# IPMI-ICNS-UKE/4d-cbct-mc

Hardware: AMD Instinct MI355X
Metric: photon histories/sec (512^3 vol, 894 proj) (higher is better)
Workload: dtype f32

## Files before the change

4d-cbct-mc_amd/csrc/engine.cpp:

```cpp
#include "engine_internal.hpp"

using namespace mcgpu;

namespace mcgpu {
namespace {
thread_local std::string g_last_error;
}
int set_error(int code, const std::string& msg) {
  g_last_error = msg.find("ERROR") == std::string::npos ? "!!ERROR!! " + msg : msg;
  return code;
}
}

extern "C" {

int mcgpu_abi_version(void) { return 1; }
void mcgpu_set_last_error_(const char* message) { (void)set_error(-1, message ? message : "unknown failure"); }
const char* mcgpu_last_error(void) { return g_last_error.c_str(); }

int mcgpu_create(const char* input_path, int device_id, mcgpu_ctx** out) {
  ABI_BEGIN
  require(input_path && out, -1, "!!ERROR!! mcgpu_create: null argument");
  knobs_warn_unknown();
  std::unique_ptr<mcgpu_ctx> c(new mcgpu_ctx);
// ... 58 lines not shown
  else if (k == "bricks_exterior") *value = ctx->dev.bricks_exterior;
  else if (k == "exterior_cylinder") *value = ctx->dev.ell_inv[0] > 0.f ? 1 : 0;
  else if (k == "sub_bricks") *value = (long long)ctx->dev.sub_n[0] * ctx->dev.sub_n[1] * ctx->dev.sub_n[2];
  else if (k == "sub_bricks_mixed") *value = ctx->dev.sub_mixed;
  else if (k == "tile_records") *value = ctx->dev.tile_rec ? 1 : 0;
  else if (k == "sub_brick_table") *value = ctx->dev.sub ? 1 : 0;
  else if (k == "segment_loop") *value = make_args(*ctx, 0).segment_loop;
  else if (k == "fast_scheduler") *value = ctx->dev.knobs.fast_sched;
  else if (k == "tiles_in_mixed_bricks") *value = ctx->dev.tiles_in_mixed_bricks;
  else if (k == "warp_field_bytes") *value = (long long)ctx->dev.warp_field_bytes;
  else if (k == "warp_field_buffer") *value = ctx->dev.dvf ? 1 : 0;
  else if (k == "correspondence_dims") *value = ctx->dev.corr_coef ? ctx->dev.corr_k : 0;
  else if (k == "blocks_per_cu") *value = ctx->dev.resident_fast;
  else if (k == "lds_bytes_fast") *value = ctx->dev.lds.total;
  else if (k == "tally_stage_bins") *value = stage_wanted(ctx->dev) ? (long long)ctx->dev.stage_bins : 0;
  else if (k == "tally_stage_capacity") *value = ctx->dev.stage_plan.cap;
  else if (k == "tally_stage_bytes") *value = (long long)ctx->dev.stage_region_bytes;
  else if (k == "tally_stage_fallback_hits") {
    unsigned long long n = 0;
    if (ctx->has_device && ctx->dev.stage_fallback) {
      HIP_TRY(hipSetDevice(ctx->dev.device_id));
      HIP_TRY(hipDeviceSynchronize());
      HIP_TRY(hipMemcpy(&n, ctx->dev.stage_fallback, 8, hipMemcpyDeviceToHost));
    }
    *value = (long long)n;
  }
  else if (k == "tally_stage_staged_hits") {
    unsigned long long n = 0;
    const size_t words = (size_t)ctx->dev.stage_plan.workgroups * ctx->dev.stage_plan.n_bins;
    if (ctx->has_device && ctx->dev.stage_counts && words != 0) {
      std::vector<unsigned int> c(words);
      HIP_TRY(hipSetDevice(ctx->dev.device_id));
      HIP_TRY(hipDeviceSynchronize());
      HIP_TRY(hipMemcpy(c.data(), ctx->dev.stage_counts, words * 4, hipMemcpyDeviceToHost));
      for (unsigned int v : c) n += v;
    }
    *value = (long long)n;
  }
// ... 67 lines not shown
  if (total_histories) *total_histories = L.total_histories;
  return 0;
  ABI_END
}

int mcgpu_advance_seed(int batch_number, unsigned long long total_histories, int seed) {
  return ranecu_advance_seed(batch_number, total_histories, seed);
}

static bool stage_wanted(const DeviceModel& D) {
  if (D.stage_cursor < 0 || D.knobs.tally_stage == 0) return false;
  if (D.knobs.tally_stage > 0) return true;
  return D.brick_count > 0 && 100LL * D.bricks_exterior >= (long long)kStageExteriorPercent * D.brick_count;
}

static void stage_prepare(mcgpu_ctx& C, TrackArgs& A, int blocks, hipStream_t stream) {
  DeviceModel& D = C.dev;
  if (D.stage_alloc_failed || blocks <= 0) return;
  const TallyStagePlan P = tally_stage_plan(4ULL * (unsigned long long)C.host.detector[0].total_pixels, A.count, (unsigned int)blocks, D.stage_bins,
                                            (unsigned int)D.knobs.stage_cap);
  if (P.n_bins == 0u || P.n_bins != D.stage_bins) return;
  const size_t counts_bytes = (size_t)blocks * P.n_bins * 4;
  try {
    if (!D.stage_fallback) D.stage_fallback = D.put(std::vector<unsigned long long>(2, 0ULL));
    if (counts_bytes > D.stage_counts_bytes) {
      if (D.stage_counts) { D.mem.free(D.stage_counts); D.stage_counts = nullptr; D.stage_counts_bytes = 0; }
      D.stage_counts = (unsigned int*)D.mem.device_bytes(counts_bytes);
      D.stage_counts_bytes = counts_bytes;
    }
    if (P.bytes > D.stage_region_bytes) {
      if (D.stage_region) { D.mem.free(D.stage_region); D.stage_region = nullptr; D.stage_region_bytes = 0; }
      D.stage_region = (unsigned long long*)D.mem.device_bytes((size_t)P.bytes);
      D.stage_region_bytes = (size_t)P.bytes;
    }
  } catch (const Error&) {
    (void)hipGetLastError();
    D.stage_alloc_failed = true;
    return;
  }
  StageArgs S{};
  S.region = D.stage_region; S.counts = D.stage_counts; S.fallback = D.stage_fallback;
  S.pixels = P.pixels; S.n_bins = P.n_bins; S.magic = P.magic; S.bin_pixels = P.bin_pixels; S.cap = P.cap;
  S.cursor = D.stage_cursor;
  if (!D.stage_fold_ready) {
    HIP_TRY(prepare_tally_fold(S));
    D.stage_fold_ready = true;
  }
  HIP_TRY(hipMemsetAsync(D.stage_counts, 0, counts_bytes, stream));
  D.stage_plan = P;
  A.stage = S;
}

int mcgpu_tally_stage_plan(const mcgpu_ctx* ctx, unsigned long long detector_words, unsigned long long histories, int workgroups, int bins,
                           unsigned long long limit, unsigned long long* out6) {
  ABI_BEGIN
  (void)ctx;
  require(out6 && workgroups > 0 && bins >= 0 && limit > 0, -1, "!!ERROR!! mcgpu_tally_stage_plan: bad argument");
  const TallyStagePlan P = tally_stage_plan(detector_words, std::min(histories, limit), (unsigned int)workgroups, (unsigned int)bins, 0u);
  out6[0] = P.n_bins; out6[1] = P.words_per_bin; out6[2] = P.bin_pixels; out6[3] = P.cap; out6[4] = P.bytes;
  out6[5] = stage_sub_launches(histories, limit);
  return 0;
  ABI_END
}

int mcgpu_tally_stage_map(unsigned long long detector_words, int bins, unsigned long long first, unsigned long long n, unsigned int* bin_out,
                          unsigned int* rel_out) {
  ABI_BEGIN
  require(bin_out && rel_out && bins >= 0 && first + n <= detector_words, -1, "!!ERROR!! mcgpu_tally_stage_map: bad argument");
  const TallyStagePlan P = tally_stage_plan(detector_words, 1, 1, (unsigned int)bins, 0u);
  require(P.n_bins != 0u, -2, "!!ERROR!! mcgpu_tally_stage_map: no staging plan for this detector");
  for (unsigned long long i = 0; i < n; ++i) {
    stage_map((unsigned int)(first + i), P.pixels, P.n_bins, P.magic, P.bin_pixels, bin_out[i], rel_out[i]);
    require(stage_unmap(bin_out[i], rel_out[i], P.pixels, P.n_bins, P.bin_pixels) == (unsigned int)(first + i), -9,
            "!!ERROR!! internal: stage_map and stage_unmap disagree");
  }
// ... 37 lines not shown
      HIP_TRY(launch_track_compat(A, (int)blocks, stream));
    } else {
      if (D.resident_fast <= 0) {
        D.resident_fast = D.knobs.blocks_per_cu > 0 ? D.knobs.blocks_per_cu : std::min(occupancy_track_fast(A), occupancy_track_fast64(A));
        if (D.resident_fast <= 0) D.resident_fast = 1;
      }
      unsigned long long resident = (unsigned long long)D.num_cus * (unsigned long long)D.resident_fast;
      resident += resident * (unsigned long long)D.knobs.grid_spare_percent / 100ULL;
      A.work_counter = D.work_counter;
      const bool staged = stage_wanted(D);
      const unsigned long long limit = staged ? D.knobs.stage_max_histories : count;
      const unsigned long long n_sub = staged ? stage_sub_launches(count, limit) : 1ULL;
      for (unsigned long long k = 0; k < n_sub; ++k) {
        stage_sub_launch(first, count, limit, k, A.first, A.count);
        const int blocks = (int)std::min((A.count + kPoolBlockThreads - 1) / kPoolBlockThreads, resident);
        HIP_TRY(hipMemsetAsync(D.work_counter, 0, (size_t)kNumCounters * kCounterStride * 8, stream));
        A.stage = StageArgs{};
        if (staged) stage_prepare(*ctx, A, blocks, stream);
        if (mode == MCGPU_MODE_FAST_STATS) {
#if defined(MC_WITH_STATS) && MC_WITH_STATS
          if (!D.stats) D.stats = D.put(std::vector<unsigned long long>(kNumStats + 3 * kWaveTrace, 0ULL));
          A.stats = D.stats;
          HIP_TRY(launch_track_stats(A, blocks, stream));
#else
          throw Error(-2, "!!ERROR!! mcgpu_launch_projection: MCGPU_MODE_FAST_STATS needs the diagnostic library (libmcgpu_amd_stats.so, MCGPU_AMD_LIB)");
#endif
        } else if (mode == MCGPU_MODE_FAST_F64) {
          HIP_TRY(launch_track_fast64(A, blocks, stream));
        } else {
          HIP_TRY(launch_track_fast(A, blocks, stream));
        }
        if (A.stage.region != nullptr) HIP_TRY(launch_tally_fold(A.stage, (unsigned int)blocks, A.image, stream));
      }
    }
  }
  HIP_TRY(hipEventRecord(D.ev_stop, stream));
  D.timed = true;
  return 0;
  ABI_END
}

int mcgpu_set_fast_schedule(mcgpu_ctx* ctx, int thresh_compton, int thresh_rayleigh, int thresh_new, int flyable_low, int swap_batch) {
  ABI_BEGIN
  require(ctx && ctx->has_device, -1, "!!ERROR!! mcgpu_set_fast_schedule: no device context");
  require(thresh_compton >= 1 && thresh_rayleigh >= 1 && thresh_new >= 1 && flyable_low >= 1 && swap_batch >= 1 && thresh_compton <= 64 &&
              thresh_rayleigh <= 64 && thresh_new <= 64 && flyable_low <= 64 && swap_batch <= 64,
          -2, "!!ERROR!! mcgpu_set_fast_schedule: thresholds are lane counts in 1..64");
// ... 313 lines not shown
```

4d-cbct-mc_amd/csrc/engine_internal.hpp:

```cpp
#pragma once
#include <hip/hip_runtime.h>

#include <algorithm>
#include <chrono>
#include <cstdarg>
#include <cstdio>
#include <cmath>
#include <cstring>
#include <map>
#include <memory>
#include <string>
#include <unordered_map>

#include "../../include/mcgpu_amd.h"
#include "knobs.hpp"
#include "device_model.hpp"
#include "ascii_device.hpp"
#include "geometry_device.hpp"
#include "image_map.hpp"

namespace mcgpu {

hipError_t launch_track_compat(const TrackArgs& args, int blocks, hipStream_t stream);
hipError_t launch_track_fast(const TrackArgs& args, int blocks, hipStream_t stream);
int occupancy_track_fast(const TrackArgs& args);
hipError_t launch_track_fast64(const TrackArgs& args, int blocks, hipStream_t stream);
int occupancy_track_fast64(const TrackArgs& args);
hipError_t launch_kat_fast64(int n, const unsigned int* u, const double* a, const double* b, const double* c, const float* dir, double* out, hipStream_t stream);
#if defined(MC_WITH_STATS) && MC_WITH_STATS
hipError_t launch_track_stats(const TrackArgs& args, int blocks, hipStream_t stream);
#endif
hipError_t prepare_tally_fold(const StageArgs& S);
hipError_t launch_tally_fold(const StageArgs& S, unsigned int workgroups, unsigned long long* image, hipStream_t stream);
hipError_t microbench_valu_issue(int num_cus, double out3[3], hipStream_t stream);
hipError_t microbench_atomic_rate(double* out, hipStream_t stream);
hipError_t microbench_copy_rate(int num_cus, double* out, hipStream_t stream);
hipError_t launch_kat_rng(int mode, int seed, int batch, int hpt, int n, float* out_dev, hipStream_t stream);
hipError_t launch_kat_streams_fast(int generator, unsigned int seed, unsigned int stream_key, unsigned long long first_id,
                                   const unsigned long long* ids_dev, int n_ids, int n_draws, unsigned int* out_dev, hipStream_t stream);
hipError_t launch_kat_math(int n, const double* x, double* l, double* e, double* s, double* c, hipStream_t stream);
hipError_t launch_kat_expf(int n, const float* x, float* e, hipStream_t stream);
hipError_t launch_kat_f32(int op, int n, const float* a, const float* b, float* out, hipStream_t stream);
hipError_t launch_warp(int nx, int ny, int nz, const unsigned char* mat, const float* dens, const float* dvf, unsigned char default_mat,
                       float default_dens, unsigned char* out_mat, float* out_dens, hipStream_t stream);
hipError_t launch_finalize(unsigned long long* image, int nx, int nz, int crop_nx, double norm, float* planes, int clear, hipStream_t stream);


int set_error(int code, const std::string& msg);
// ... 69 lines not shown
  int has_exterior = 0, bricks_exterior = 0;
  float objbox_lo[3] = {0, 0, 0}, objbox_hi[3] = {0, 0, 0};
  float ell_c[2] = {0, 0}, ell_inv[2] = {0, 0};
  LdsLayout lds;
  TrackCold* cold = nullptr;
  TrackCold cold_host;
  unsigned long long* dose_voxels = nullptr;
  unsigned long long* dose_materials = nullptr;
  size_t dose_roi_voxels = 0;
  int dose_flags = 0;
  SourcePose* src_all = nullptr;
  DetectorPose* det_all = nullptr;
  int resident_fast = 0;
  unsigned long long* stats = nullptr;
  unsigned long long* work_counter = nullptr;
  int stage_cursor = -1;
  unsigned int stage_bins = 0;
  unsigned long long* stage_region = nullptr;
  size_t stage_region_bytes = 0;
  unsigned int* stage_counts = nullptr;
  size_t stage_counts_bytes = 0;
  unsigned long long* stage_fallback = nullptr;
  bool stage_alloc_failed = false, stage_fold_ready = false;
  TallyStagePlan stage_plan{};
  unsigned long long* scratch_image = nullptr;
  float *woodcock = nullptr, *mfp = nullptr, *mfp_tot = nullptr;
  float* wood_coarse = nullptr;
  int sig_shift = -1;
  int sched[5] = {40, 12, 44, 12, 40};
  bool sched_set = false;
  struct Knobs {
    int exterior_mode = 3;
    bool compat_stats = false;
    int compat_thresh[4] = {-1, -1, -1, -1};
    int blocks_per_cu = 0;
    int grid_spare_percent = 0;
    int sched_override[5] = {-1, -1, -1, -1, -1};
    int slot_trade = 3, hold_q = 6;
// ... 64 lines not shown
```

4d-cbct-mc_amd/csrc/knobs.cpp:

```cpp
#include <cstdio>
#include <cstdlib>
#include <cstring>
#include <mutex>
#include <string>

#include "host_model.hpp"
#include "knobs.hpp"
#include "../../include/mcgpu_amd.h"

extern char** environ;

namespace mcgpu {

const KnobSpec kKnobs[] = {
    {"MCGPU_AMD_LIB", 's', 'P', "4d-cbct-mc_amd/libmcgpu_amd.so", "library the Python mirror loads (engine.py: load_library); A/B builds and the diagnostic library go through it"},
    {"MCGPU_FAST_SCHED", 'i', 'K', "0", "FAST scheduler: 0 per-wave pools, 1 workgroup-level pool (bit-identical, 14-23 % slower; fixed when the model is uploaded)"},
    {"MCGPU_SEGMENT_LOOP", 'i', 'K', "-1", "flight segment as an inner loop: 1 on, 0 off, -1 host heuristic (tile records, or >= 20 electron shells per material on average)"},
    {"MCGPU_TILE_RECORDS", 'i', 'K', "auto", "16-byte tile records (two to four palette entries + a 64-bit mask per 4x4x4 tile) as second level of the u8 volume: 1 on, 0 off; default on when the tiles of the mixed bricks exceed 8 MiB (thorax +9 %, CT-textured +29 %); identical tallies"},
    {"MCGPU_SUB_BRICKS", 'i', 'K', "0", "4-bit sub-brick codes as second level (superseded by the tile records; kept for A/B)"},
    {"MCGPU_MAX_BRICKS", 'i', 'K', "fit", "upper limit of the LDS brick grid (a coarser grid frees LDS); default: what is left of 80 KB after the tables"},
    {"MCGPU_NO_BRACKETS", 'b', 'K', "off", "no cross-section brackets in LDS: every material change asks the exact table"},
    {"MCGPU_NO_EXTERIOR", 'b', 'K', "off", "no analytic exterior hop / source entry: delta-tracking everywhere, as the reference"},
    {"MCGPU_EXTERIOR_MODE", 'i', 'K', "3", "bit 0: exterior hop of photons in flight, bit 1: analytic source entry"},
    {"MCGPU_NO_ELLIPSE", 'b', 'K', "off", "object region = bounding box only (no elliptic cylinder; default: cylinder when >= 5 % of the bricks lie outside it)"},
    {"MCGPU_THRESH_COMPTON", 'i', 'K', "40", "lanes a Compton batch waits for (1..64); setting any schedule knob also switches the scan's autotune off"},
    {"MCGPU_THRESH_RAYLEIGH", 'i', 'K', "12", "lanes a Rayleigh batch waits for"},
    {"MCGPU_THRESH_NEW", 'i', 'K', "44", "lanes a tally + source batch waits for"},
    {"MCGPU_FLYABLE_LOW", 'i', 'K', "12", "below this many flyable histories the wave drains its pending kinds"},
    {"MCGPU_SWAP_BATCH", 'i', 'K', "40", "lanes that may park before the next scheduling point"},
    {"MCGPU_HOLD_Q", 'i', 'K', "6", "a flight segment ends when all but hold_q/16 of its starting lanes have parked (0..15)"},
    {"MCGPU_SLOT_TRADE", 'i', 'K', "3", "bit 0: trade slots for flyable histories, bit 1: for the service batches"},
    {"MCGPU_NO_AUTOTUNE", 'b', 'K', "off", "scan driver: keep the default schedule instead of probing the three presets on 6e6 histories"},
    {"MCGPU_BLOCKS_PER_CU", 'i', 'K', "occupancy", "resident FAST workgroups per CU (default: what the occupancy query reports, normally 2)"},
    {"MCGPU_GRID_SPARE_PERCENT", 'i', 'K', "0", "extra workgroups beyond the resident grid, in percent"},
    {"MCGPU_TALLY_STAGE", 'i', 'K', "-1", "FAST kernels: detector hits are staged per (workgroup, bin) with plain stores and folded into the image by a second kernel (tally_fold.hip) instead of one 64-bit atomic each (bit-identical): 1 on, 0 off, -1 on where at least 50 % of the bricks are exterior (`bricks_exterior` / `brick_count`: Catphan 96 % +3 %; CIRS 26 %, thorax 43 %: 1.7-6 % slower, left on the atomics) ; in every setting only where the cursor table ((bins + 1) x 4 B) fits what the LDS image leaves of 80 KB -- otherwise the launch runs the direct atomics, also when forced on (`geti(\"tally_stage_bins\")` = 0 says so)"},
    {"MCGPU_TALLY_STAGE_MAX_HISTORIES", 'i', 'K', "134217728", "staged launches above this many histories are split into sub-launches, each followed by its fold (the staging buffer takes about 10 bytes per history of a sub-launch)"},
    {"MCGPU_COMPAT_THRESH_COMPTON", 'i', 'K', "-1", "COMPAT kernel: lanes a Compton batch waits for (-1: built-in 32, or 48 when the materials average >= 20 electron shells)"},
    {"MCGPU_COMPAT_THRESH_RAYLEIGH", 'i', 'K', "-1", "COMPAT kernel: Rayleigh batch threshold (built-in 4 / 8)"},
    {"MCGPU_COMPAT_THRESH_NEW", 'i', 'K', "-1", "COMPAT kernel: tally + source batch threshold (built-in 24 / 16)"},
    {"MCGPU_COMPAT_THRESH_TAKE", 'i', 'K', "-1", "COMPAT kernel: lanes whose parked history could fly while their register history cannot, to exchange the two (built-in 2)"},
    {"MCGPU_COMPAT_STATS", 'i', 'K', "0", "COMPAT kernel section counters (diagnostic build -DMC_COMPAT_STATS only)"},
    {"MCGPU_IGNORE_VOXBIN", 'b', 'H', "off", "parse geometry.vox(.gz) even when a newer geometry.voxbin sidecar lies beside it"},
    {"MCGPU_ASCII_HOST", 'b', 'H', "off", "format the reference's ASCII projection files on the host threads instead of the device (A/B)"},
    {"MCGPU_ASCII_WRITERS", 'i', 'H', "slots", "ASCII files in flight (1..MCGPU_ASCII_SLOTS)"},
    {"MCGPU_PINNED_COHERENT", 'b', 'H', "off", "coherent pinned host buffers for the downloads (default: non-coherent)"},
    {"MCGPU_FDK_DIRECT_RAMP", 'b', 'H', "off", "FDK ramp filter as a direct LDS convolution instead of hipFFT"},
    {"MCGPU_CORRESPONDENCE_SLAB", 'i', 'H', "4194304", "device fit of a correspondence model: field elements per slab (T slabs of 4 bytes per element are staged on the device at a time)"},
    {"MCGPU_REDUCE", 's', 'H', "auto", "multi-device tally sum: `rccl` = one ncclReduce per projection; default: tally exchange, else projection sharding"},
    {"MCGPU_RCCL_LIBRARY", 's', 'H', "librccl.so.1", "RCCL library the reduction route opens with dlopen"},
    {"MCGPU_EXCHANGE_POLICY", 'i', 'H', "1", "tally exchange: 1 the owner of a projection rotates over the ranks, 0 rank 0 owns every projection"},
// ... 57 lines not shown
```

4d-cbct-mc_amd/csrc/model_device.cpp:

```cpp
#include "engine_internal.hpp"

namespace mcgpu {

std::vector<float> coarse_woodcock(const HostModel& H) {
  const int nv = H.mat.num_values, nc = (nv + (1 << kWoodShift) - 1) >> kWoodShift;
  const double e0 = (double)H.mat.e0, de = 1.0 / (double)H.mat.ide;
  std::vector<float> out((size_t)nc, 0.f);
  for (int c = 0; c < nc; ++c) {
    double lo = 1.0e30;
    for (int i = c << kWoodShift; i < std::min(nv, (c + 1) << kWoodShift); ++i) {
      const double x = (double)H.mat.woodcock[i].x, y = (double)H.mat.woodcock[i].y;
      lo = std::min(lo, std::min(x + (e0 + i * de) * y, x + (e0 + (i + 1) * de) * y));
    }
    out[(size_t)c] = (float)(lo * (1.0 - 1.0e-6));
  }
  return out;
}

static void mark_exterior_region(const HostModel& H, DeviceModel& D, const std::vector<unsigned char>& object, bool have_background,
                                 std::vector<unsigned char>& exterior) {
  const int k = D.brick_shift, nvx[3] = {H.voxels.n[0], H.voxels.n[1], H.voxels.n[2]};
  exterior.assign((size_t)D.brick_count, 0);
  D.has_exterior = 0;
  D.bricks_exterior = 0;
// ... 757 lines not shown
      wmax = std::max(wmax, std::max((hi - m) / m, (m - lo) / m));
    }
    B.w[c] = (float)std::min(wmax * 1.001 + 1e-5, 1e30);
  }
  return B;
}

static void lay_out_lds_and_brackets(const HostModel& H, DeviceModel& D, const std::vector<float>& tot) {
  const LdsPlan P = plan_lds(H, D, D.brick_bytes);
  D.sig_shift = -1;
  if (!knob_set("MCGPU_NO_BRACKETS") && D.nmat > 0)
    for (int shift = 6; shift <= 12 && D.sig_shift < 0; ++shift)
      if (lay_out_lds(P, shift).total <= kLdsPerWorkgroup) D.sig_shift = shift;
  D.lds = lay_out_lds(P, D.sig_shift);
  {
    const TallyStagePlan S = tally_stage_plan(4ULL * (unsigned long long)H.detector[0].total_pixels, 1, 1, 0, 0);
    const int bytes = ((int)(S.n_bins + 1u) * 4 + 15) / 16 * 16;
    D.stage_cursor = -1;
    D.stage_bins = 0;
    if (S.n_bins != 0u && D.lds.total + bytes <= kLdsPerWorkgroup) {
      D.stage_cursor = D.lds.total;
      D.stage_bins = S.n_bins;
      D.lds.total += bytes;
    }
  }
  if (D.sig_shift < 0) return;
  const SigmaBrackets B = sigma_brackets(H, tot, D.nmat, D.sig_shift);
  D.cold_host.sig_mid = D.put(B.mid);
  D.cold_host.sig_w = D.put(B.w);
}

static void upload_dose_tallies(const HostModel& H, DeviceModel& D) {
  const SimConfig& cfg = H.cfg;
  if (cfg.flag_material_dose == 1) {
// ... 236 lines not shown
```

4d-cbct-mc_amd/csrc/tally_fold.hip:

```cpp
#include <hip/hip_runtime.h>

#include "tally_stage.hpp"

namespace mcgpu {
namespace {

constexpr int kFoldThreads = 1024;
extern __shared__ __attribute__((aligned(16))) unsigned long long fold_lds[];

__device__ __forceinline__ void fold_add(unsigned long long record, unsigned int words) {
  const unsigned int rel = (unsigned int)(record >> 32);
  if (rel < words) atomicAdd(fold_lds + rel, record & 0xFFFFFFFFULL);
}

__global__ __launch_bounds__(kFoldThreads) void tally_stage_fold(const StageArgs S, const unsigned int workgroups, unsigned long long* __restrict__ image) {
  const unsigned int bin = blockIdx.x, words = 4u * S.bin_pixels;
  for (unsigned int i = threadIdx.x; i < words; i += kFoldThreads) fold_lds[i] = 0ULL;
  __syncthreads();
  const unsigned int wave = (unsigned int)__builtin_amdgcn_readfirstlane((int)(threadIdx.x >> 6)), lane = threadIdx.x & 63u;
  constexpr unsigned int kWaves = kFoldThreads / 64;
  constexpr unsigned int kGroup = 4, kDeep = 4;
  for (unsigned int g0 = wave; g0 < workgroups; g0 += 64u * kWaves) {
    const unsigned int g_mine = g0 + lane * kWaves;
    const unsigned int n_mine = g_mine < workgroups ? min(S.counts[(size_t)g_mine * S.n_bins + bin], S.cap) : 0u;
    for (unsigned int l0 = 0; l0 < 64u && g0 + l0 * kWaves < workgroups; l0 += kGroup) {
      ulonglong2 r[kGroup][kDeep];
      unsigned int n[kGroup];
      const unsigned long long* src[kGroup];
#pragma unroll
      for (unsigned int u = 0; u < kGroup; ++u) {
        n[u] = (unsigned int)__builtin_amdgcn_readlane((int)n_mine, (int)(l0 + u));
        const unsigned int g = min(g0 + (l0 + u) * kWaves, workgroups - 1u);
        src[u] = S.region + (size_t)(g * S.n_bins + bin) * S.cap;
        const ulonglong2* const src2 = reinterpret_cast<const ulonglong2*>(src[u]);
#pragma unroll
        for (unsigned int j = 0; j < kDeep; ++j) {
          const unsigned int i = lane + 64u * j;
          r[u][j] = make_ulonglong2(~0ULL, ~0ULL);
          if (i < (n[u] >> 1)) r[u][j] = src2[i];
        }
      }
#pragma unroll
      for (unsigned int u = 0; u < kGroup; ++u) {
#pragma unroll
        for (unsigned int j = 0; j < kDeep; ++j) {
          fold_add(r[u][j].x, words);
          fold_add(r[u][j].y, words);
        }
        const ulonglong2* const src2 = reinterpret_cast<const ulonglong2*>(src[u]);
        for (unsigned int i = lane + 64u * kDeep; i < (n[u] >> 1); i += 64u) {
          const ulonglong2 a = src2[i];
          fold_add(a.x, words);
          fold_add(a.y, words);
        }
        if ((n[u] & 1u) != 0u && lane == 0u) fold_add(src[u][n[u] - 1u], words);
      }
    }
  }
  __syncthreads();
  for (unsigned int i = threadIdx.x; i < words; i += kFoldThreads) {
    const unsigned long long v = fold_lds[i];
    if (v == 0ULL) continue;
    const unsigned int w = stage_unmap(bin, i, S.pixels, S.n_bins, S.bin_pixels);
    if (w != 0xFFFFFFFFu) image[w] += v;
  }
}

}

hipError_t prepare_tally_fold(const StageArgs& S) {
  const size_t lds = (size_t)4 * S.bin_pixels * 8;
  if (lds <= 64 * 1024) return hipSuccess;
  return hipFuncSetAttribute(reinterpret_cast<const void*>(&tally_stage_fold), hipFuncAttributeMaxDynamicSharedMemorySize, (int)lds);
}

hipError_t launch_tally_fold(const StageArgs& S, unsigned int workgroups, unsigned long long* image, hipStream_t stream) {
  hipLaunchKernelGGL(tally_stage_fold, dim3(S.n_bins), dim3(kFoldThreads), (size_t)4 * S.bin_pixels * 8, stream, S, workgroups, image);
  return hipGetLastError();
}

}
```

4d-cbct-mc_amd/csrc/tally_stage.hpp:

```cpp
#pragma once
#include <cstdint>

#if defined(__HIPCC__)
#define MC_STAGE_HD __host__ __device__
#else
#define MC_STAGE_HD
#endif

namespace mcgpu {

constexpr unsigned int kStageRun = 64;
constexpr unsigned int kStageRunsPerBin = 64;
constexpr int kStageExteriorPercent = 50;
constexpr unsigned int kStageCapSlack = 16;
constexpr unsigned int kStageWorkgroupSlack = 2u * 16u * 256u;

struct TallyStagePlan {
  unsigned int pixels;
  unsigned int n_bins;
  unsigned int bin_pixels;
  unsigned int words_per_bin;
  unsigned int magic;
  unsigned int cap;
  unsigned int workgroups;
// ... 46 lines not shown
MC_STAGE_HD inline unsigned int stage_unmap(unsigned int bin, unsigned int rel, unsigned int pixels, unsigned int n_bins, unsigned int bin_pixels) {
  const unsigned int plane = (rel >= bin_pixels ? 1u : 0u) + (rel >= 2u * bin_pixels ? 1u : 0u) + (rel >= 3u * bin_pixels ? 1u : 0u);
  const unsigned int off = rel - plane * bin_pixels;
  const unsigned long long pixel = ((unsigned long long)(off / kStageRun) * n_bins + bin) * kStageRun + (off % kStageRun);
  return pixel < pixels ? plane * pixels + (unsigned int)pixel : 0xFFFFFFFFu;
}

inline void stage_sub_launch(unsigned long long first, unsigned long long count, unsigned long long limit, unsigned long long k, unsigned long long& sub_first,
                             unsigned long long& sub_count) {
  const unsigned long long at = k * limit;
  sub_first = first + (at < count ? at : count);
  sub_count = at < count ? (count - at < limit ? count - at : limit) : 0ULL;
}
inline unsigned long long stage_sub_launches(unsigned long long count, unsigned long long limit) { return count == 0 ? 1ULL : (count + limit - 1) / limit; }

struct StageArgs {
  unsigned long long* region;
  unsigned int* counts;
  unsigned long long* fallback;
  unsigned int pixels, n_bins, magic, bin_pixels, cap;
  int cursor;
};

}
```

4d-cbct-mc_amd/engine.py:

```python
from __future__ import annotations

import ctypes as C
import os
from pathlib import Path
from typing import Optional, Sequence

import numpy as np

MODE_FAST, MODE_COMPAT, MODE_FAST_STATS, MODE_FAST_F64 = 0, 1, 2, 3
_MODES = {"fast": MODE_FAST, "compat": MODE_COMPAT, "stats": MODE_FAST_STATS, "fast64": MODE_FAST_F64, MODE_FAST: MODE_FAST,
          MODE_COMPAT: MODE_COMPAT, MODE_FAST_STATS: MODE_FAST_STATS, MODE_FAST_F64: MODE_FAST_F64}

LIB_PATH = Path(os.environ.get("MCGPU_AMD_LIB", Path(__file__).resolve().parent / "libmcgpu_amd.so"))
EXE_PATH = Path(__file__).resolve().parent / "MC-GPU_v1.3.x"

ABI_SYMBOLS = (
    "mcgpu_abi_version", "mcgpu_knob_table", "mcgpu_last_error", "mcgpu_create", "mcgpu_clone", "mcgpu_destroy", "mcgpu_config_i64", "mcgpu_config_f64",
    "mcgpu_host_table", "mcgpu_projection_file_name", "mcgpu_image_words", "mcgpu_launch_shape", "mcgpu_advance_seed",
    "mcgpu_launch_projection", "mcgpu_tally_stage_plan", "mcgpu_tally_stage_map", "mcgpu_tally_stage_sub_launch", "mcgpu_scheduler_stats", "mcgpu_scheduler_stats_ex", "mcgpu_last_kernel_ms", "mcgpu_clear_image", "mcgpu_run_projection",
    "mcgpu_write_projection", "mcgpu_format_projection", "mcgpu_write_formatted_projection", "mcgpu_dose_info", "mcgpu_dose_read", "mcgpu_dose_clear", "mcgpu_write_dose_report",
    "mcgpu_finalize_projection", "mcgpu_finalize_projection_host", "mcgpu_stack_create", "mcgpu_stack_append", "mcgpu_stack_write_slice", "mcgpu_stack_finish",
    "mcgpu_stack_read", "mcgpu_normalize_stack", "mcgpu_run_scan", "mcgpu_run_scan_multi", "mcgpu_set_projection_angles", "mcgpu_set_geometry_arrays",
    "mcgpu_warp_volume", "mcgpu_warp_geometry", "mcgpu_map_image", "mcgpu_set_geometry_image",
    "mcgpu_correspondence_set", "mcgpu_correspondence_fit", "mcgpu_correspondence_predict", "mcgpu_warp_geometry_signal", "mcgpu_correspondence_clear",
    "mcgpu_write_voxel_file", "mcgpu_write_voxel_binary", "mcgpu_kat_rng", "mcgpu_kat_rng_streams", "mcgpu_microbench", "mcgpu_kat_math", "mcgpu_kat_expf", "mcgpu_kat_f32", "mcgpu_kat_fast64", "mcgpu_kat_tile_records", "mcgpu_fdk_reconstruct", "mcgpu_forward_project", "mcgpu_forward_project_context", "mcgpu_rooster4d_reconstruct", "mcgpu_rooster4d_stage", "mcgpu_set_fast_schedule", "mcgpu_reload_env_knobs",
    "mcgpu_exchange_shared_bytes", "mcgpu_exchange_card_bytes", "mcgpu_exchange_create", "mcgpu_exchange_card", "mcgpu_exchange_connect",
    "mcgpu_exchange_connect_local", "mcgpu_exchange_probe", "mcgpu_exchange_owner", "mcgpu_exchange_begin", "mcgpu_exchange_submit", "mcgpu_exchange_collect",
    "mcgpu_exchange_stats", "mcgpu_exchange_destroy", "mcgpu_copy_to_host",
    "mcgpu_rccl_create", "mcgpu_rccl_reduce_u64", "mcgpu_rccl_destroy",
)


class ScanOptions(C.Structure):
    _fields_ = [("struct_size", C.c_uint), ("mode", C.c_int), ("first_projection", C.c_int), ("num_projections", C.c_int),
# ... 59 lines not shown
    lib.mcgpu_knob_table.restype = C.c_size_t
    lib.mcgpu_create.argtypes = [cp, ci, C.POINTER(vp)]
    lib.mcgpu_clone.argtypes = [vp, ci, C.POINTER(vp)]
    lib.mcgpu_destroy.argtypes = [vp]
    lib.mcgpu_destroy.restype = None
    lib.mcgpu_config_i64.argtypes = [vp, cp, C.POINTER(C.c_longlong)]
    lib.mcgpu_config_f64.argtypes = [vp, cp, C.POINTER(C.c_double)]
    lib.mcgpu_host_table.argtypes = [vp, cp, C.POINTER(vp), C.POINTER(C.c_size_t)]
    lib.mcgpu_projection_file_name.argtypes = [vp, ci, cp, C.c_size_t]
    lib.mcgpu_image_words.argtypes = [vp, C.POINTER(C.c_size_t)]
    lib.mcgpu_launch_shape.argtypes = [cull, ci, ci, C.POINTER(ci), C.POINTER(ci), C.POINTER(cull)]
    lib.mcgpu_advance_seed.argtypes = [ci, cull, ci]
    lib.mcgpu_launch_projection.argtypes = [vp, ci, ci, ci, cull, cull, ci, vp, vp]
    lib.mcgpu_tally_stage_plan.argtypes = [vp, cull, cull, ci, ci, cull, C.POINTER(cull)]
    lib.mcgpu_tally_stage_map.argtypes = [cull, ci, cull, cull, vp, vp]
    lib.mcgpu_tally_stage_sub_launch.argtypes = [cull, cull, cull, cull, C.POINTER(cull), C.POINTER(cull)]
    lib.mcgpu_last_kernel_ms.argtypes = [vp, C.POINTER(C.c_float)]
    lib.mcgpu_scheduler_stats.argtypes = [vp, C.POINTER(cull), ci]
    lib.mcgpu_scheduler_stats_ex.argtypes = [vp, C.POINTER(cull), ci, ci]
    lib.mcgpu_clear_image.argtypes = [vp, vp, vp]
    lib.mcgpu_run_projection.argtypes = [vp, ci, ci, ci, cull, cull, ci, vp, C.POINTER(C.c_double), C.POINTER(cull)]
    lib.mcgpu_write_projection.argtypes = [vp, ci, vp, cull, C.c_double, cp]
    lib.mcgpu_format_projection.argtypes = [vp, vp, cull, ci, vp]
    lib.mcgpu_write_formatted_projection.argtypes = [vp, ci, ci, cull, C.c_double, cp]
    lib.mcgpu_dose_info.argtypes = [vp, C.POINTER(ci), C.POINTER(ci), C.POINTER(C.c_size_t)]
    lib.mcgpu_dose_read.argtypes = [vp, vp, vp]
    lib.mcgpu_dose_clear.argtypes = [vp]
    lib.mcgpu_write_dose_report.argtypes = [vp, vp, vp, cull, C.c_double, cp, C.c_size_t]
    lib.mcgpu_finalize_projection.argtypes = [vp, vp, cull, ci, vp, ci, vp]
    lib.mcgpu_finalize_projection_host.argtypes = [vp, vp, cull, ci, vp]
# ... 62 lines not shown


def tally_stage_plan(detector_words: int, histories: int, workgroups: int, bins: int = 0, limit: int = 1 << 27, ctx=None) -> dict:
    out = (C.c_ulonglong * 6)()
    _check(load_library().mcgpu_tally_stage_plan(ctx.h if ctx is not None else None, int(detector_words), int(histories), int(workgroups), int(bins), int(limit), out))
    return dict(zip(("bins", "words_per_bin", "bin_pixels", "capacity", "bytes", "sub_launches"), (int(v) for v in out)))


def tally_stage_map(detector_words: int, bins: int = 0, first: int = 0, n: Optional[int] = None):
    n = int(detector_words) - int(first) if n is None else int(n)
    b, r = np.empty(n, np.uint32), np.empty(n, np.uint32)
    _check(load_library().mcgpu_tally_stage_map(int(detector_words), int(bins), int(first), n, b.ctypes.data, r.ctypes.data))
    return b, r


def tally_stage_sub_launch(first: int, count: int, limit: int, k: int):
    f, c = C.c_ulonglong(), C.c_ulonglong()
    _check(load_library().mcgpu_tally_stage_sub_launch(int(first), int(count), int(limit), int(k), C.byref(f), C.byref(c)))
    return f.value, c.value


def advance_seed(batch_number: int, total_histories: int, seed: int) -> int:
    return load_library().mcgpu_advance_seed(batch_number, int(total_histories), seed)


def write_voxel_file(path, n, spacing_cm, material_zyx: np.ndarray, density_zyx: np.ndarray, gzip: bool = True):
    m = np.ascontiguousarray(material_zyx, dtype=np.uint8)
    d = np.ascontiguousarray(density_zyx, dtype=np.float32)
    assert m.size == d.size == int(n[0]) * int(n[1]) * int(n[2])
    _check(load_library().mcgpu_write_voxel_file(str(path).encode(), (C.c_int * 3)(*map(int, n)), (C.c_float * 3)(*map(float, spacing_cm)),
# ... 596 lines not shown
```

include/mcgpu_amd.h:

```cpp
#ifndef MCGPU_AMD_H_
#define MCGPU_AMD_H_

#include <stddef.h>
#include <stdint.h>

#ifdef __cplusplus
extern "C" {
#endif

typedef struct mcgpu_ctx mcgpu_ctx;

#define MCGPU_MODE_FAST 0
#define MCGPU_MODE_COMPAT 1
#define MCGPU_MODE_FAST_STATS 2
#define MCGPU_MODE_FAST_F64 3

int mcgpu_abi_version(void);
size_t mcgpu_knob_table(char *buf, size_t cap);
const char *mcgpu_last_error(void);

int mcgpu_create(const char *input_path, int device_id, mcgpu_ctx **out);
void mcgpu_destroy(mcgpu_ctx *ctx);
int mcgpu_clone(const mcgpu_ctx *src, int device_id, mcgpu_ctx **out);

// ... 5 lines not shown
int mcgpu_projection_file_name(const mcgpu_ctx *ctx, int p, char *buf, size_t buf_bytes);

int mcgpu_image_words(const mcgpu_ctx *ctx, size_t *words);

int mcgpu_launch_shape(unsigned long long histories, int threads_per_block, int histories_per_thread, int *blocks,
                       int *hpt_out, unsigned long long *total_histories);

int mcgpu_advance_seed(int batch_number, unsigned long long total_histories, int seed);

int mcgpu_launch_projection(mcgpu_ctx *ctx, int p, int mode, int seed, unsigned long long first, unsigned long long count,
                            int hpt, void *image_dev, void *hip_stream);
int mcgpu_tally_stage_plan(const mcgpu_ctx *ctx, unsigned long long detector_words, unsigned long long histories, int workgroups,
                           int bins, unsigned long long limit, unsigned long long *out6);
int mcgpu_tally_stage_map(unsigned long long detector_words, int bins, unsigned long long first, unsigned long long n,
                          unsigned int *bin_out, unsigned int *rel_out);
int mcgpu_tally_stage_sub_launch(unsigned long long first, unsigned long long count, unsigned long long limit, unsigned long long k,
                                 unsigned long long *sub_first, unsigned long long *sub_count);
int mcgpu_last_kernel_ms(mcgpu_ctx *ctx, float *ms);
int mcgpu_scheduler_stats(mcgpu_ctx *ctx, unsigned long long *out8, int reset);
int mcgpu_set_fast_schedule(mcgpu_ctx *ctx, int thresh_compton, int thresh_rayleigh, int thresh_new, int flyable_low, int swap_batch);
int mcgpu_reload_env_knobs(mcgpu_ctx *ctx);
int mcgpu_scheduler_stats_ex(mcgpu_ctx *ctx, unsigned long long *out, int capacity, int reset);
int mcgpu_copy_to_host(mcgpu_ctx *ctx, const void *src_dev, void *dst_host, size_t bytes, void *hip_stream);

int mcgpu_clear_image(mcgpu_ctx *ctx, void *image_dev, void *hip_stream);

int mcgpu_run_projection(mcgpu_ctx *ctx, int p, int mode, int seed, unsigned long long first, unsigned long long count, int hpt,
                         uint64_t *image_host, double *kernel_seconds, unsigned long long *histories_done);

int mcgpu_write_projection(mcgpu_ctx *ctx, int p, const uint64_t *image_host, unsigned long long total_histories, double seconds,
// ... 223 lines not shown
```

Measured before the change: 28.12 billion.

## Fold staged tallies with one bin per CU using 32-bit LDS counters

The staging plan now uses one bin per compute unit instead of the default plan. Each bin is folded in 32-bit LDS counters, and any 32-bit wraps are recorded in a carry list and added to the image as 64-bit carries. The fold kernel also zeroes the work dispensers, so the next staged launch on the same stream skips its memset, and the per-launch memset of the stage counts is removed. This aims to cut fold-kernel count, LDS footprint and launch overhead, at the cost of more complex carry handling and an ordering assumption for graph replay.

```diff
diff --git a/4d-cbct-mc_amd/csrc/engine.cpp b/4d-cbct-mc_amd/csrc/engine.cpp
--- a/4d-cbct-mc_amd/csrc/engine.cpp
+++ b/4d-cbct-mc_amd/csrc/engine.cpp
@@ -96,14 +96,16 @@
   else if (k == "blocks_per_cu") *value = ctx->dev.resident_fast;
   else if (k == "lds_bytes_fast") *value = ctx->dev.lds.total;
   else if (k == "tally_stage_bins") *value = stage_wanted(ctx->dev) ? (long long)ctx->dev.stage_bins : 0;
+  else if (k == "tally_stage_fold_bits") *value = stage_wanted(ctx->dev) ? (ctx->dev.stage_narrow ? 32 : 64) : 0;
   else if (k == "tally_stage_capacity") *value = ctx->dev.stage_plan.cap;
   else if (k == "tally_stage_bytes") *value = (long long)ctx->dev.stage_region_bytes;
-  else if (k == "tally_stage_fallback_hits") {
+  else if (k == "tally_stage_fallback_hits" || k == "tally_stage_fold_carries" || k == "tally_stage_fold_carries_direct") {
     unsigned long long n = 0;
+    const int at = k == "tally_stage_fallback_hits" ? 0 : (k == "tally_stage_fold_carries" ? 1 : 2);
     if (ctx->has_device && ctx->dev.stage_fallback) {
       HIP_TRY(hipSetDevice(ctx->dev.device_id));
       HIP_TRY(hipDeviceSynchronize());
-      HIP_TRY(hipMemcpy(&n, ctx->dev.stage_fallback, 8, hipMemcpyDeviceToHost));
+      HIP_TRY(hipMemcpy(&n, ctx->dev.stage_fallback + at, 8, hipMemcpyDeviceToHost));
     }
     *value = (long long)n;
   }
@@ -201,7 +203,7 @@
   return D.brick_count > 0 && 100LL * D.bricks_exterior >= (long long)kStageExteriorPercent * D.brick_count;
 }
 
-static void stage_prepare(mcgpu_ctx& C, TrackArgs& A, int blocks, hipStream_t stream) {
+static void stage_prepare(mcgpu_ctx& C, TrackArgs& A, int blocks) {
   DeviceModel& D = C.dev;
   if (D.stage_alloc_failed || blocks <= 0) return;
   const TallyStagePlan P = tally_stage_plan(4ULL * (unsigned long long)C.host.detector[0].total_pixels, A.count, (unsigned int)blocks, D.stage_bins,
@@ -209,7 +211,7 @@
   if (P.n_bins == 0u || P.n_bins != D.stage_bins) return;
   const size_t counts_bytes = (size_t)blocks * P.n_bins * 4;
   try {
-    if (!D.stage_fallback) D.stage_fallback = D.put(std::vector<unsigned long long>(2, 0ULL));
+    if (!D.stage_fallback) D.stage_fallback = D.put(std::vector<unsigned long long>(4, 0ULL));
     if (counts_bytes > D.stage_counts_bytes) {
       if (D.stage_counts) { D.mem.free(D.stage_counts); D.stage_counts = nullptr; D.stage_counts_bytes = 0; }
       D.stage_counts = (unsigned int*)D.mem.device_bytes(counts_bytes);
@@ -230,10 +232,9 @@
   S.pixels = P.pixels; S.n_bins = P.n_bins; S.magic = P.magic; S.bin_pixels = P.bin_pixels; S.cap = P.cap;
   S.cursor = D.stage_cursor;
   if (!D.stage_fold_ready) {
-    HIP_TRY(prepare_tally_fold(S));
+    HIP_TRY(prepare_tally_fold());
     D.stage_fold_ready = true;
   }
-  HIP_TRY(hipMemsetAsync(D.stage_counts, 0, counts_bytes, stream));
   D.stage_plan = P;
   A.stage = S;
 }
@@ -246,6 +247,16 @@
   const TallyStagePlan P = tally_stage_plan(detector_words, std::min(histories, limit), (unsigned int)workgroups, (unsigned int)bins, 0u);
   out6[0] = P.n_bins; out6[1] = P.words_per_bin; out6[2] = P.bin_pixels; out6[3] = P.cap; out6[4] = P.bytes;
   out6[5] = stage_sub_launches(histories, limit);
+  return 0;
+  ABI_END
+}
+
+int mcgpu_tally_stage_engine_bins(unsigned long long detector_words, int cus, int* out2) {
+  ABI_BEGIN
+  require(out2 && cus >= 0, -1, "!!ERROR!! mcgpu_tally_stage_engine_bins: bad argument");
+  bool narrow = false;
+  out2[0] = (int)stage_engine_bins(detector_words, (unsigned int)cus, narrow);
+  out2[1] = narrow ? 32 : 64;
   return 0;
   ABI_END
 }
@@ -313,9 +324,10 @@
       for (unsigned long long k = 0; k < n_sub; ++k) {
         stage_sub_launch(first, count, limit, k, A.first, A.count);
         const int blocks = (int)std::min((A.count + kPoolBlockThreads - 1) / kPoolBlockThreads, resident);
-        HIP_TRY(hipMemsetAsync(D.work_counter, 0, (size_t)kNumCounters * kCounterStride * 8, stream));
+        if (!(D.dispensers_clean && D.dispensers_stream == stream)) HIP_TRY(hipMemsetAsync(D.work_counter, 0, (size_t)kNumCounters * kCounterStride * 8, stream));
+        D.dispensers_clean = false;
         A.stage = StageArgs{};
-        if (staged) stage_prepare(*ctx, A, blocks, stream);
+        if (staged) stage_prepare(*ctx, A, blocks);
         if (mode == MCGPU_MODE_FAST_STATS) {
 #if defined(MC_WITH_STATS) && MC_WITH_STATS
           if (!D.stats) D.stats = D.put(std::vector<unsigned long long>(kNumStats + 3 * kWaveTrace, 0ULL));
@@ -329,7 +341,13 @@
         } else {
           HIP_TRY(launch_track_fast(A, blocks, stream));
         }
-        if (A.stage.region != nullptr) HIP_TRY(launch_tally_fold(A.stage, (unsigned int)blocks, A.image, stream));
+        if (A.stage.region != nullptr) {
+          require(D.stage_plan.workgroups == (unsigned int)blocks, -9, "!!ERROR!! internal: the staging plan is not of the grid launched");
+          const bool zero_dispensers = mode != MCGPU_MODE_FAST_STATS;
+          HIP_TRY(launch_tally_fold(A.stage, D.stage_narrow, (unsigned int)blocks, A.image, zero_dispensers ? D.work_counter : nullptr, stream));
+          D.dispensers_clean = zero_dispensers;
+          D.dispensers_stream = stream;
+        }
       }
     }
   }
diff --git a/4d-cbct-mc_amd/csrc/engine_internal.hpp b/4d-cbct-mc_amd/csrc/engine_internal.hpp
--- a/4d-cbct-mc_amd/csrc/engine_internal.hpp
+++ b/4d-cbct-mc_amd/csrc/engine_internal.hpp
@@ -30,8 +30,9 @@
 #if defined(MC_WITH_STATS) && MC_WITH_STATS
 hipError_t launch_track_stats(const TrackArgs& args, int blocks, hipStream_t stream);
 #endif
-hipError_t prepare_tally_fold(const StageArgs& S);
-hipError_t launch_tally_fold(const StageArgs& S, unsigned int workgroups, unsigned long long* image, hipStream_t stream);
+hipError_t prepare_tally_fold();
+hipError_t launch_tally_fold(const StageArgs& S, bool narrow, unsigned int workgroups, unsigned long long* image, unsigned long long* dispensers,
+                             hipStream_t stream);
 hipError_t microbench_valu_issue(int num_cus, double out3[3], hipStream_t stream);
 hipError_t microbench_atomic_rate(double* out, hipStream_t stream);
 hipError_t microbench_copy_rate(int num_cus, double* out, hipStream_t stream);
@@ -131,14 +132,18 @@
   int resident_fast = 0;
   unsigned long long* stats = nullptr;
   unsigned long long* work_counter = nullptr;
+  bool dispensers_clean = false;
+  hipStream_t dispensers_stream = nullptr;
   int stage_cursor = -1;
   unsigned int stage_bins = 0;
+  bool stage_narrow = false;
   unsigned long long* stage_region = nullptr;
   size_t stage_region_bytes = 0;
   unsigned int* stage_counts = nullptr;
   size_t stage_counts_bytes = 0;
   unsigned long long* stage_fallback = nullptr;
-  bool stage_alloc_failed = false, stage_fold_ready = false;
+  bool stage_alloc_failed = false;
+  bool stage_fold_ready = false;
   TallyStagePlan stage_plan{};
   unsigned long long* scratch_image = nullptr;
   float *woodcock = nullptr, *mfp = nullptr, *mfp_tot = nullptr;
diff --git a/4d-cbct-mc_amd/csrc/knobs.cpp b/4d-cbct-mc_amd/csrc/knobs.cpp
--- a/4d-cbct-mc_amd/csrc/knobs.cpp
+++ b/4d-cbct-mc_amd/csrc/knobs.cpp
@@ -33,7 +33,7 @@
     {"MCGPU_NO_AUTOTUNE", 'b', 'K', "off", "scan driver: keep the default schedule instead of probing the three presets on 6e6 histories"},
     {"MCGPU_BLOCKS_PER_CU", 'i', 'K', "occupancy", "resident FAST workgroups per CU (default: what the occupancy query reports, normally 2)"},
     {"MCGPU_GRID_SPARE_PERCENT", 'i', 'K', "0", "extra workgroups beyond the resident grid, in percent"},
-    {"MCGPU_TALLY_STAGE", 'i', 'K', "-1", "FAST kernels: detector hits are staged per (workgroup, bin) with plain stores and folded into the image by a second kernel (tally_fold.hip) instead of one 64-bit atomic each (bit-identical): 1 on, 0 off, -1 on where at least 50 % of the bricks are exterior (`bricks_exterior` / `brick_count`: Catphan 96 % +3 %; CIRS 26 %, thorax 43 %: 1.7-6 % slower, left on the atomics) ; in every setting only where the cursor table ((bins + 1) x 4 B) fits what the LDS image leaves of 80 KB -- otherwise the launch runs the direct atomics, also when forced on (`geti(\"tally_stage_bins\")` = 0 says so)"},
+    {"MCGPU_TALLY_STAGE", 'i', 'K', "-1", "FAST kernels: detector hits are staged per (workgroup, bin) with plain stores and folded into the image by a second kernel (tally_fold.hip) instead of one 64-bit atomic each (bit-identical): 1 on, 0 off, -1 on where at least 50 % of the bricks are exterior (`bricks_exterior` / `brick_count`: Catphan 96 % +3 %; CIRS 26 %, thorax 43 %: 1.7-6 % slower, left on the atomics) ; in every setting only where the cursor table ((bins + 1) x 4 B) fits what the LDS image leaves of 80 KB -- otherwise the launch runs the direct atomics, also when forced on (`geti(\"tally_stage_bins\")` = 0 says so); the plan holds one bin per compute unit, folded in 32-bit LDS counters with carries, or the default plan and 64-bit counters where such a bin does not fit the fold's LDS (`geti(\"tally_stage_fold_bits\")` = 32 / 64); a staged launch that follows a staged launch of its context in the same stream issues no fill -- decided as the launch is enqueued, so launches captured into a graph must not be replayed in another order; `geti(\"tally_stage_fold_carries\")` / `geti(\"tally_stage_fold_carries_direct\")` count the 32-bit wraps carried and those that found the carry list full"},
     {"MCGPU_TALLY_STAGE_MAX_HISTORIES", 'i', 'K', "134217728", "staged launches above this many histories are split into sub-launches, each followed by its fold (the staging buffer takes about 10 bytes per history of a sub-launch)"},
     {"MCGPU_COMPAT_THRESH_COMPTON", 'i', 'K', "-1", "COMPAT kernel: lanes a Compton batch waits for (-1: built-in 32, or 48 when the materials average >= 20 electron shells)"},
     {"MCGPU_COMPAT_THRESH_RAYLEIGH", 'i', 'K', "-1", "COMPAT kernel: Rayleigh batch threshold (built-in 4 / 8)"},
diff --git a/4d-cbct-mc_amd/csrc/model_device.cpp b/4d-cbct-mc_amd/csrc/model_device.cpp
--- a/4d-cbct-mc_amd/csrc/model_device.cpp
+++ b/4d-cbct-mc_amd/csrc/model_device.cpp
@@ -795,10 +795,14 @@
       if (lay_out_lds(P, shift).total <= kLdsPerWorkgroup) D.sig_shift = shift;
   D.lds = lay_out_lds(P, D.sig_shift);
   {
-    const TallyStagePlan S = tally_stage_plan(4ULL * (unsigned long long)H.detector[0].total_pixels, 1, 1, 0, 0);
+    const unsigned long long words = 4ULL * (unsigned long long)H.detector[0].total_pixels;
+    bool narrow = false;
+    const unsigned int bins = stage_engine_bins(words, (unsigned int)D.num_cus, narrow);
+    const TallyStagePlan S = tally_stage_plan(words, 1, 1, bins, 0);
     const int bytes = ((int)(S.n_bins + 1u) * 4 + 15) / 16 * 16;
     D.stage_cursor = -1;
     D.stage_bins = 0;
+    D.stage_narrow = narrow;
     if (S.n_bins != 0u && D.lds.total + bytes <= kLdsPerWorkgroup) {
       D.stage_cursor = D.lds.total;
       D.stage_bins = S.n_bins;
diff --git a/4d-cbct-mc_amd/csrc/tally_fold.hip b/4d-cbct-mc_amd/csrc/tally_fold.hip
--- a/4d-cbct-mc_amd/csrc/tally_fold.hip
+++ b/4d-cbct-mc_amd/csrc/tally_fold.hip
@@ -1,25 +1,59 @@
 #include <hip/hip_runtime.h>
 
+#include "device_model.hpp"
 #include "tally_stage.hpp"
 
 namespace mcgpu {
 namespace {
 
 constexpr int kFoldThreads = 1024;
+constexpr unsigned long long kCarry = 1ULL << 32;
 extern __shared__ __attribute__((aligned(16))) unsigned long long fold_lds[];
 
-__device__ __forceinline__ void fold_add(unsigned long long record, unsigned int words) {
-  const unsigned int rel = (unsigned int)(record >> 32);
-  if (rel < words) atomicAdd(fold_lds + rel, record & 0xFFFFFFFFULL);
-}
+template <bool kNarrow>
+struct FoldBin {
+  unsigned int bin, words;
+  const StageArgs& S;
+  unsigned long long* image;
+  __device__ __forceinline__ unsigned int* narrow_counters() const { return reinterpret_cast<unsigned int*>(fold_lds); }
+  __device__ __forceinline__ unsigned int* control() const { return narrow_counters() + words; }
+  __device__ __forceinline__ unsigned int* carries() const { return control() + 2; }
 
-__global__ __launch_bounds__(kFoldThreads) void tally_stage_fold(const StageArgs S, const unsigned int workgroups, unsigned long long* __restrict__ image) {
+  __device__ __forceinline__ void add(unsigned long long record) const {
+    const unsigned int rel = (unsigned int)(record >> 32), v = (unsigned int)record;
+    if (rel >= words) return;
+    if (!kNarrow) {
+      atomicAdd(fold_lds + rel, (unsigned long long)v);
+      return;
+    }
+    const unsigned int old = atomicAdd(narrow_counters() + rel, v);
+    if (old + v < old) {
+      const unsigned int k = atomicAdd(control(), 1u);
+      if (k < kFoldCarrySlots) {
+        carries()[k] = rel;
+      } else {
+        control()[1] = 1u;
+        const unsigned int w = stage_unmap(bin, rel, S.pixels, S.n_bins, S.bin_pixels);
+        if (w != 0xFFFFFFFFu) atomicAdd(image + w, kCarry);
+      }
+    }
+  }
+};
+
+template <bool kNarrow>
+__global__ __launch_bounds__(kFoldThreads) void tally_stage_fold(const StageArgs S, const unsigned int workgroups, unsigned long long* __restrict__ image,
+                                                                 unsigned long long* __restrict__ dispensers) {
   const unsigned int bin = blockIdx.x, words = 4u * S.bin_pixels;
-  for (unsigned int i = threadIdx.x; i < words; i += kFoldThreads) fold_lds[i] = 0ULL;
+  const FoldBin<kNarrow> B{bin, words, S, image};
+  if (kNarrow) {
+    for (unsigned int i = threadIdx.x; i < words + 2u; i += kFoldThreads) B.narrow_counters()[i] = 0u;
+  } else {
+    for (unsigned int i = threadIdx.x; i < words; i += kFoldThreads) fold_lds[i] = 0ULL;
+  }
   __syncthreads();
   const unsigned int wave = (unsigned int)__builtin_amdgcn_readfirstlane((int)(threadIdx.x >> 6)), lane = threadIdx.x & 63u;
   constexpr unsigned int kWaves = kFoldThreads / 64;
-  constexpr unsigned int kGroup = 4, kDeep = 4;
+  constexpr unsigned int kGroup = 4, kDeep = kNarrow ? 5 : 4;
   for (unsigned int g0 = wave; g0 < workgroups; g0 += 64u * kWaves) {
     const unsigned int g_mine = g0 + lane * kWaves;
     const unsigned int n_mine = g_mine < workgroups ? min(S.counts[(size_t)g_mine * S.n_bins + bin], S.cap) : 0u;
@@ -44,38 +78,69 @@
       for (unsigned int u = 0; u < kGroup; ++u) {
 #pragma unroll
         for (unsigned int j = 0; j < kDeep; ++j) {
-          fold_add(r[u][j].x, words);
-          fold_add(r[u][j].y, words);
+          B.add(r[u][j].x);
+          B.add(r[u][j].y);
         }
         const ulonglong2* const src2 = reinterpret_cast<const ulonglong2*>(src[u]);
         for (unsigned int i = lane + 64u * kDeep; i < (n[u] >> 1); i += 64u) {
           const ulonglong2 a = src2[i];
-          fold_add(a.x, words);
-          fold_add(a.y, words);
+          B.add(a.x);
+          B.add(a.y);
         }
-        if ((n[u] & 1u) != 0u && lane == 0u) fold_add(src[u][n[u] - 1u], words);
+        if ((n[u] & 1u) != 0u && lane == 0u) B.add(src[u][n[u] - 1u]);
       }
     }
   }
   __syncthreads();
-  for (unsigned int i = threadIdx.x; i < words; i += kFoldThreads) {
-    const unsigned long long v = fold_lds[i];
-    if (v == 0ULL) continue;
-    const unsigned int w = stage_unmap(bin, i, S.pixels, S.n_bins, S.bin_pixels);
-    if (w != 0xFFFFFFFFu) image[w] += v;
+  if (kNarrow) {
+    const unsigned int* const counter = B.narrow_counters();
+    const bool list_full = B.control()[1] != 0u;
+    for (unsigned int i = threadIdx.x; i < words; i += kFoldThreads) {
+      const unsigned int v = counter[i];
+      if (v == 0u) continue;
+      const unsigned int w = stage_unmap(bin, i, S.pixels, S.n_bins, S.bin_pixels);
+      if (w == 0xFFFFFFFFu) continue;
+      if (list_full) atomicAdd(image + w, (unsigned long long)v);
+      else image[w] += v;
+    }
+    const unsigned int wraps = B.control()[0], n_carry = min(wraps, kFoldCarrySlots);
+    if (wraps != 0u && threadIdx.x == 0u) {
+      atomicAdd(S.fallback + 1, (unsigned long long)wraps);
+      if (wraps > n_carry) atomicAdd(S.fallback + 2, (unsigned long long)(wraps - n_carry));
+    }
+    if (n_carry != 0u) {
+      __threadfence();
+      __syncthreads();
+      for (unsigned int k = threadIdx.x; k < n_carry; k += kFoldThreads) {
+        const unsigned int w = stage_unmap(bin, B.carries()[k], S.pixels, S.n_bins, S.bin_pixels);
+        if (w != 0xFFFFFFFFu) atomicAdd(image + w, kCarry);
+      }
+    }
+  } else {
+    for (unsigned int i = threadIdx.x; i < words; i += kFoldThreads) {
+      const unsigned long long v = fold_lds[i];
+      if (v == 0ULL) continue;
+      const unsigned int w = stage_unmap(bin, i, S.pixels, S.n_bins, S.bin_pixels);
+      if (w != 0xFFFFFFFFu) image[w] += v;
+    }
   }
+  if (dispensers != nullptr && bin == 0u && threadIdx.x < (unsigned int)kNumCounters) dispensers[threadIdx.x * (unsigned int)kCounterStride] = 0ULL;
 }
 
 }
 
-hipError_t prepare_tally_fold(const StageArgs& S) {
-  const size_t lds = (size_t)4 * S.bin_pixels * 8;
-  if (lds <= 64 * 1024) return hipSuccess;
-  return hipFuncSetAttribute(reinterpret_cast<const void*>(&tally_stage_fold), hipFuncAttributeMaxDynamicSharedMemorySize, (int)lds);
+hipError_t prepare_tally_fold() {
+  const hipError_t e = hipFuncSetAttribute(reinterpret_cast<const void*>(&tally_stage_fold<true>), hipFuncAttributeMaxDynamicSharedMemorySize, (int)kFoldLdsLimit);
+  if (e != hipSuccess) return e;
+  return hipFuncSetAttribute(reinterpret_cast<const void*>(&tally_stage_fold<false>), hipFuncAttributeMaxDynamicSharedMemorySize, (int)kFoldLdsLimit);
 }
 
-hipError_t launch_tally_fold(const StageArgs& S, unsigned int workgroups, unsigned long long* image, hipStream_t stream) {
-  hipLaunchKernelGGL(tally_stage_fold, dim3(S.n_bins), dim3(kFoldThreads), (size_t)4 * S.bin_pixels * 8, stream, S, workgroups, image);
+hipError_t launch_tally_fold(const StageArgs& S, bool narrow, unsigned int workgroups, unsigned long long* image, unsigned long long* dispensers,
+                             hipStream_t stream) {
+  const unsigned int lds = stage_fold_lds_bytes(S.bin_pixels, narrow);
+  if (lds > kFoldLdsLimit) return hipErrorInvalidValue;
+  if (narrow) hipLaunchKernelGGL(tally_stage_fold<true>, dim3(S.n_bins), dim3(kFoldThreads), (size_t)lds, stream, S, workgroups, image, dispensers);
+  else hipLaunchKernelGGL(tally_stage_fold<false>, dim3(S.n_bins), dim3(kFoldThreads), (size_t)lds, stream, S, workgroups, image, dispensers);
   return hipGetLastError();
 }
 
diff --git a/4d-cbct-mc_amd/csrc/tally_stage.hpp b/4d-cbct-mc_amd/csrc/tally_stage.hpp
--- a/4d-cbct-mc_amd/csrc/tally_stage.hpp
+++ b/4d-cbct-mc_amd/csrc/tally_stage.hpp
@@ -84,6 +84,25 @@
 }
 inline unsigned long long stage_sub_launches(unsigned long long count, unsigned long long limit) { return count == 0 ? 1ULL : (count + limit - 1) / limit; }
 
+constexpr unsigned int kFoldLdsLimit = 128u * 1024u;
+constexpr unsigned int kFoldCarrySlots = 1022;
+inline unsigned int stage_fold_lds_bytes(unsigned int bin_pixels, bool narrow) {
+  return narrow ? 4u * bin_pixels * 4u + (kFoldCarrySlots + 2u) * 4u : 4u * bin_pixels * 8u;
+}
+inline unsigned int stage_engine_bins(unsigned long long detector_words, unsigned int cus, bool& narrow) {
+  narrow = false;
+  const unsigned long long runs = (detector_words / 4ULL + kStageRun - 1) / kStageRun;
+  if (cus == 0u || runs == 0ULL) return 0u;
+  unsigned int bins = cus;
+  if (runs < 8ULL * cus) {
+    const unsigned long long per_bin = (runs + cus - 1) / cus;
+    bins = (unsigned int)((runs + per_bin - 1) / per_bin);
+  }
+  const TallyStagePlan P = tally_stage_plan(detector_words, 1, 1, bins, 0);
+  narrow = P.n_bins != 0u && stage_fold_lds_bytes(P.bin_pixels, true) <= kFoldLdsLimit;
+  return narrow ? bins : 0u;
+}
+
 struct StageArgs {
   unsigned long long* region;
   unsigned int* counts;
diff --git a/4d-cbct-mc_amd/engine.py b/4d-cbct-mc_amd/engine.py
--- a/4d-cbct-mc_amd/engine.py
+++ b/4d-cbct-mc_amd/engine.py
@@ -17,7 +17,7 @@
 ABI_SYMBOLS = (
     "mcgpu_abi_version", "mcgpu_knob_table", "mcgpu_last_error", "mcgpu_create", "mcgpu_clone", "mcgpu_destroy", "mcgpu_config_i64", "mcgpu_config_f64",
     "mcgpu_host_table", "mcgpu_projection_file_name", "mcgpu_image_words", "mcgpu_launch_shape", "mcgpu_advance_seed",
-    "mcgpu_launch_projection", "mcgpu_tally_stage_plan", "mcgpu_tally_stage_map", "mcgpu_tally_stage_sub_launch", "mcgpu_scheduler_stats", "mcgpu_scheduler_stats_ex", "mcgpu_last_kernel_ms", "mcgpu_clear_image", "mcgpu_run_projection",
+    "mcgpu_launch_projection", "mcgpu_tally_stage_plan", "mcgpu_tally_stage_map", "mcgpu_tally_stage_engine_bins", "mcgpu_tally_stage_sub_launch", "mcgpu_scheduler_stats", "mcgpu_scheduler_stats_ex", "mcgpu_last_kernel_ms", "mcgpu_clear_image", "mcgpu_run_projection",
     "mcgpu_write_projection", "mcgpu_format_projection", "mcgpu_write_formatted_projection", "mcgpu_dose_info", "mcgpu_dose_read", "mcgpu_dose_clear", "mcgpu_write_dose_report",
     "mcgpu_finalize_projection", "mcgpu_finalize_projection_host", "mcgpu_stack_create", "mcgpu_stack_append", "mcgpu_stack_write_slice", "mcgpu_stack_finish",
     "mcgpu_stack_read", "mcgpu_normalize_stack", "mcgpu_run_scan", "mcgpu_run_scan_multi", "mcgpu_set_projection_angles", "mcgpu_set_geometry_arrays",
@@ -107,6 +107,7 @@
     lib.mcgpu_launch_projection.argtypes = [vp, ci, ci, ci, cull, cull, ci, vp, vp]
     lib.mcgpu_tally_stage_plan.argtypes = [vp, cull, cull, ci, ci, cull, C.POINTER(cull)]
     lib.mcgpu_tally_stage_map.argtypes = [cull, ci, cull, cull, vp, vp]
+    lib.mcgpu_tally_stage_engine_bins.argtypes = [cull, ci, C.POINTER(ci)]
     lib.mcgpu_tally_stage_sub_launch.argtypes = [cull, cull, cull, cull, C.POINTER(cull), C.POINTER(cull)]
     lib.mcgpu_last_kernel_ms.argtypes = [vp, C.POINTER(C.c_float)]
     lib.mcgpu_scheduler_stats.argtypes = [vp, C.POINTER(cull), ci]
@@ -199,6 +200,12 @@
     return b, r
 
 
+def tally_stage_engine_bins(detector_words: int, cus: int):
+    out = (C.c_int * 2)()
+    _check(load_library().mcgpu_tally_stage_engine_bins(int(detector_words), int(cus), out))
+    return int(out[0]), int(out[1])
+
+
 def tally_stage_sub_launch(first: int, count: int, limit: int, k: int):
     f, c = C.c_ulonglong(), C.c_ulonglong()
     _check(load_library().mcgpu_tally_stage_sub_launch(int(first), int(count), int(limit), int(k), C.byref(f), C.byref(c)))
diff --git a/include/mcgpu_amd.h b/include/mcgpu_amd.h
--- a/include/mcgpu_amd.h
+++ b/include/mcgpu_amd.h
@@ -43,6 +43,7 @@
                            int bins, unsigned long long limit, unsigned long long *out6);
 int mcgpu_tally_stage_map(unsigned long long detector_words, int bins, unsigned long long first, unsigned long long n,
                           unsigned int *bin_out, unsigned int *rel_out);
+int mcgpu_tally_stage_engine_bins(unsigned long long detector_words, int cus, int *out2);
 int mcgpu_tally_stage_sub_launch(unsigned long long first, unsigned long long count, unsigned long long limit, unsigned long long k,
                                  unsigned long long *sub_first, unsigned long long *sub_count);
 int mcgpu_last_kernel_ms(mcgpu_ctx *ctx, float *ms);
```

Measured after the change: 28.54 billion, median of 6. 1.5% higher.
